# wei-zeng98/piano-a2s

Measured on AMD Instinct MI355X. Metric: training clips/sec (12 s, 5-bar), higher is better.
Workload: dtype f32

## Files before the change

### include/a2s.h

```cpp
#ifndef A2S_H
#define A2S_H
#include <stddef.h>
#include <stdint.h>
#ifdef __cplusplus
extern "C" {
#endif

#define A2S_OK 0
#define A2S_ERR_ARG (-1)
#define A2S_ERR_HIP (-2)
#define A2S_ERR_WORKSPACE (-3)

const char* a2s_last_error(void);
int a2s_version(void);
long long a2s_launch_count(void);

int a2s_gemm_f32(void* stream, int M, int N, int K, float alpha, const float* A, long sAm, long sAk,
                 const float* B, long sBk, long sBn, float beta, float* C, long ldc, const float* bias, int act,
                 int batch, long bsA, long bsB, long bsC, int splitk, float* workspace, size_t workspace_bytes);
int a2s_gemm_f32_affine(void* stream, int M, int N, int K, float alpha, const float* A, long sAm, long sAk, const float* B, long sBk,
                        long sBn, float beta, float* C, long ldc, const float* bias, int act, int batch, long bsA, long bsB, long bsC,
                        int splitk, float* workspace, size_t workspace_bytes, const float* a_scale, const float* a_shift, int a_period,
                        const float* b_scale, const float* b_shift, int b_period);
int a2s_gemm_f32_bnstats(void* stream, int M, int N, int K, const float* A, long sAm, long sAk, const float* B, long sBk, long sBn, float* C, long ldc,
// ... 14 lines not shown
int a2s_linear_wgrad(void* stream, int M, int N, int K, const float* dz, long ldz, const float* y, long lda, float* G, long ldg, const float* scale,
                     const float* shift, int period, const float* dz_absmax, const float* y_absmax, float* workspace, size_t workspace_bytes);
size_t a2s_linear_wgrad_ws_bytes(int M, int K);
int a2s_linear_wgrad_eligible(int M, int N, int K, int period);
size_t a2s_linear_dgrad_ws_bytes(int N, int K);
int a2s_linear_dgrad_blocks(int M);
int a2s_linear_dgrad_eligible(int M, int N, int K, int period);
int a2s_absmax(void* stream, const float* x, long n, float* out);
int a2s_gemm_bnstats_blocks(int M, int period);
size_t a2s_gemm_workspace_bytes(int M, int N, int batch, int splitk);
int a2s_gemm_pick_splitk(int M, int N, int K, int batch);
void a2s_gemm_debug_tile(int cfg);
int a2s_debug_set(const char* key, int value);
int a2s_debug_get(const char* key);
int a2s_env_check(void);
int a2s_persist_abort_latch(void* device_word);

int a2s_conv3x3(void* stream, const float* x, const float* w, float* y, const float* in_scale, const float* in_shift,
                float* stat_partial, int B, int T, int F, int Cin, int Cout, int flip, float* workspace);
int a2s_conv3x3_ranged(void* stream, const float* x, const float* w, float* y, const float* in_scale, const float* in_shift, const float* in_absmax,
                       float* stat_partial, float* out_absmax, int B, int T, int F, int Cin, int Cout, float* workspace);
int a2s_conv3x3_stat_blocks(int B, int T, int F, int Cin);
int a2s_conv3x3_dgrad_bnstats(void* stream, const float* dy, const float* w, float* g, const float* yl, const float* yl_mean, const float* yl_invstd,
                              const float* yl_scale, const float* yl_shift, float* stat_partial, int B, int T, int F, int Cin, int Cout,
                              float* workspace);
int a2s_bn_bwd_from_partial(void* stream, const float* g, const float* x, const float* mean, const float* invstd, const float* scale, const float* shift,
                            float* dgamma, float* dbeta, float* dx , const float* partial, int nblocks, float* c12, long rows, int C, int F);
int a2s_conv3x3_dgrad_bnstats_scaled(void* stream, const float* dy, const float* w, float* g, const float* yl, const float* yl_mean, const float* yl_invstd,
                                     const float* yl_scale, const float* yl_shift, float* stat_partial, int B, int T, int F, int Cin, int Cout,
                                     float* workspace, const float* dy_absmax);
// ... 182 lines not shown
```

### piano_a2s_amd/csrc/a2s_api.hip

```cpp
#define A2S_SWITCHES_IMPL
#include "a2s_internal.h"

thread_local char a2s_err_msg[512] = {0};
long long a2s_launch_counter = 0;

#define ST ((hipStream_t)stream)

extern "C" {

const char* a2s_last_error(void) { return a2s_err_msg; }
int a2s_version(void) { return 1; }
long long a2s_launch_count(void) { return __atomic_load_n(&a2s_launch_counter, __ATOMIC_RELAXED); }

int a2s_gemm_f32(void* stream, int M, int N, int K, float alpha, const float* A, long sAm, long sAk, const float* B, long sBk,
                 long sBn, float beta, float* C, long ldc, const float* bias, int act, int batch, long bsA, long bsB, long bsC,
                 int splitk, float* workspace, size_t workspace_bytes) {
    return a2s_gemm_impl(ST, M, N, K, alpha, A, sAm, sAk, B, sBk, sBn, beta, C, ldc, bias, act, batch, bsA, bsB, bsC, splitk,
                         workspace, workspace_bytes);
}
int a2s_gemm_f32_affine(void* stream, int M, int N, int K, float alpha, const float* A, long sAm, long sAk, const float* B, long sBk,
                        long sBn, float beta, float* C, long ldc, const float* bias, int act, int batch, long bsA, long bsB, long bsC,
                        int splitk, float* workspace, size_t workspace_bytes, const float* a_scale, const float* a_shift, int a_period,
                        const float* b_scale, const float* b_shift, int b_period) {
    return a2s_gemm_affine_impl(ST, M, N, K, alpha, A, sAm, sAk, B, sBk, sBn, beta, C, ldc, bias, act, batch, bsA, bsB, bsC, splitk,
// ... 40 lines not shown
int a2s_gemm_f32_bnstats(void* stream, int M, int N, int K, const float* A, long sAm, long sAk, const float* B, long sBk, long sBn, float* C, long ldc,
                         const float* y, const float* mean, const float* invstd, const float* scale, const float* shift, int period, float* partial) {
    return a2s_gemm_affine_impl(ST, M, N, K, 1.f, A, sAm, sAk, B, sBk, sBn, 0.f, C, ldc, nullptr, 0, 1, 0, 0, 0, 1, nullptr, 0,
                                nullptr, nullptr, 0, nullptr, nullptr, 0, y, mean, invstd, scale, shift, partial, period, 0, nullptr, nullptr);
}
int a2s_gemm_bnstats_blocks(int M, int period) { return a2s_cdiv(M, 128) * a2s_gemm_bnstats_slots(period); }
size_t a2s_gemm_workspace_bytes(int M, int N, int batch, int splitk) { return a2s_gemm_workspace_bytes_impl(M, N, batch, splitk); }
int a2s_gemm_pick_splitk(int M, int N, int K, int batch) { return a2s_gemm_pick_splitk_impl(M, N, K, batch); }
void a2s_gemm_debug_tile(int cfg) { a2s_gemm_debug_tile_impl(cfg); }
size_t a2s_note_step_workspace_floats(int H, int E) { return a2s_note_step_workspace_floats_impl(H, E); }
int a2s_debug_set(const char* key, int value) {
    if (!key) return A2S_ERR_ARG;
    const int id = a2s_switch_find(key);
    if (id >= 0) { a2s_switch_store(id, value); return A2S_OK; }
    if (!strcmp(key, "gemm_tile")) { a2s_gemm_debug_tile_impl(value); return A2S_OK; }
    snprintf(a2s_err_msg, sizeof(a2s_err_msg), "a2s_debug_set: unknown key %s", key);
    return A2S_ERR_ARG;
}
int a2s_env_check(void) {
    if (const char* e = a2s_switch_env_error()) A2S_FAIL(A2S_ERR_ARG, "%s: expected a decimal number >= 0", e);
    return A2S_OK;
}

int a2s_persist_abort_latch(void* device_word) { a2s_persist_latch_set(device_word); return A2S_OK; }

int a2s_debug_get(const char* key) {
    if (!key) return -1;
    const int id = a2s_switch_find(key);
    if (id == A2S_SW_attn_pair_fused_rows) return a2s_attn_pair_fused_rows();
    if (id >= 0) return a2s_sw((a2s_switch)id);
    if (!strcmp(key, "attn_pair_launches")) return (int)a2s_attn_pair_launches();
    if (!strcmp(key, "attn_pair_bwd_launches")) return (int)a2s_attn_pair_bwd_launches();
    if (!strcmp(key, "dec_mid_launches")) return a2s_dec_mid_launches();
    if (!strcmp(key, "dec_persist_launches")) return a2s_dec_persist_launches();
    if (!strcmp(key, "edit_distance_launches")) return (int)a2s_edit_distance_launches();
    if (!strcmp(key, "device_cus")) return a2s_device_geometry().cus;
    if (!strcmp(key, "device_xccs")) return a2s_device_geometry().xccs;
    return -1;
}

int a2s_conv3x3(void* stream, const float* x, const float* w, float* y, const float* in_scale, const float* in_shift,
                float* stat_partial, int B, int T, int F, int Cin, int Cout, int flip, float* workspace) {
    return a2s_conv3x3_impl(ST, x, w, y, in_scale, in_shift, stat_partial, B, T, F, Cin, Cout, flip, workspace, nullptr, nullptr, nullptr, nullptr, nullptr, nullptr,
                            nullptr, nullptr);
}
int a2s_conv3x3_ranged(void* stream, const float* x, const float* w, float* y, const float* in_scale, const float* in_shift, const float* in_absmax,
                       float* stat_partial, float* out_absmax, int B, int T, int F, int Cin, int Cout, float* workspace) {
    return a2s_conv3x3_impl(ST, x, w, y, in_scale, in_shift, stat_partial, B, T, F, Cin, Cout, 0, workspace, nullptr, nullptr, nullptr, nullptr, nullptr, nullptr,
// ... 243 lines not shown
```

### piano_a2s_amd/csrc/a2s_bwd.hip

```cpp
#include "a2s_internal.h"

__global__ __launch_bounds__(256) void log_softmax_bwd_rows(const float* __restrict__ g, const float* __restrict__ y,
                                                            long outer_stride, int inner, float* __restrict__ dx,
                                                            int R, int V, int n_outer, int time_major) {
    const int row = blockIdx.x * 4 + (threadIdx.x >> 6), lane = threadIdx.x & 63;
    if (row >= R) return;
    const int ob = row / inner, in = row % inner;
    const float* gr = g + (long)ob * outer_stride + (long)in * V;
    const float* yr = y + (long)ob * outer_stride + (long)in * V;
    float s = 0.f;
    for (int j = lane; j < V; j += 64) s += gr[j];
    s = wave_sum(s);
    const long orow = time_major ? ((long)in * n_outer + ob) : row;
    for (int j = lane; j < V; j += 64) dx[orow * V + j] = gr[j] - expf(yr[j]) * s;
}

int a2s_log_softmax_bwd_rows_impl(hipStream_t st, const float* g, const float* y, long outer_stride, int inner, float* dx,
                                  int R, int V, int n_outer, int time_major) {
    hipLaunchKernelGGL(log_softmax_bwd_rows, dim3(a2s_cdiv(R, 4)), dim3(256), 0, st, g, y, outer_stride, inner, dx, R, V, n_outer, time_major);
    A2S_CHECK_LAUNCH("log_softmax_bwd_rows");
    return A2S_OK;
}

__global__ void gru_gates_bwd(const float* __restrict__ dh_a, long lda, const float* __restrict__ dh_b, long ldb,
// ... 225 lines not shown

struct AttnPairBwdStep { const int* clip_order; const int* clip_rank; int n_clips; int n_active; int step; int G; int chunk; };
static int attn_pair_bwd_sweep(hipStream_t st, const a2s_note_dec_bwd_args& au, const a2s_note_dec_bwd_args& al, int s, AttnPairBwdStep& p);
static int attn_pair_bwd_combine(hipStream_t st, const a2s_note_dec_bwd_args& a, int s, const AttnPairBwdStep& p);

static int note_bwd_step_rows(const a2s_note_dec_bwd_args& a, int s) { return (a.row_list && a.n_rows_active) ? a.n_rows_active[s] : a.R; }
static thread_local int t_pair_rows_limit = -1;
struct PairRowsLimit { PairRowsLimit(int v) { t_pair_rows_limit = v; } ~PairRowsLimit() { t_pair_rows_limit = -1; } };
static bool note_bwd_step_fused(const a2s_note_dec_bwd_args& a, int s) {
    const void* ptrs[] = {a.dgi_all, a.dgh_all, a.dq_all, a.dx, a.dh, a.w_ih, a.w_hh, a.attn_w};
    const int n = note_bwd_step_rows(a, s);
    if (t_pair_rows_limit >= 0 && n > t_pair_rows_limit) return false;
    return n > 0 && a2s_dec_step_fusable(n, a.H, a.E, 173, ptrs, 8, a.step_ws, a.step_ws_floats);
}

static int note_bwd_step(hipStream_t st, const a2s_note_dec_bwd_args& a, int s, int& cur, bool mid, int part, const AttnPairBwdStep* pair) {
    const int H2 = 2 * a.H, ldx = a.E + H2, R = a.R;
    const bool fused = note_bwd_step_fused(a, s);
    a2s_attn_rows rows_v = {a.clip_order, a.clip_rank, a.row_until, a.n_clips > 0 ? a.n_clips : R, a.n_active ? a.n_active[s] : 0, s};
    const a2s_attn_rows* rows = a.n_active ? &rows_v : nullptr;
    float* dh_in = a.dh + (long)cur * R * H2;
    float* dh_out = a.dh + (long)(cur ^ 1) * R * H2;
    if (fused) {
        const int nrows = note_bwd_step_rows(a, s);
        int rc = a2s_note_step_fused_bwd(st, a, s, dh_in, dh_out, rows, nrows, nrows < R ? a.row_list : nullptr);
        if (rc) return rc;
        cur ^= 1;
        return A2S_OK;
    }
    int gM = R, gB = 1;
    long gS = 0;
    if (a.m_active && a.n_clips > 0 && a2s_prefix_rows_ok(a.m_active[s], a.n_clips)) { gM = a.m_active[s]; gB = R / a.n_clips; gS = a.n_clips; }
    const float* dos = a.do_all + (long)s * R * 2 * H2;
    float* dgi = a.dgi_all + (long)s * R * 3 * H2;
    float* dgh = a.dgh_all + (long)s * R * 3 * H2;
    float* dxs = a.dx + (long)s * R * ldx;
    int rc = A2S_OK;
    if (part != 2) {
        rc = a2s_gru_gates_bwd_impl(st, dh_in, H2, dos, 2 * H2, a.gates + (long)s * R * 4 * H2, a.h + (long)s * R * H2, H2,
                                    dgi, 3 * H2, dgh, 3 * H2, nullptr, 0, dh_out, H2, R, H2);
        if (rc) return rc;
        if (mid) {
            const int nrows = note_bwd_step_rows(a, s);
            rc = a2s_note_step_mid_bwd(st, a, s, dh_out, nrows, nrows < R ? a.row_list : nullptr);
        } else {
            rc = a2s_gemm_impl(st, gM, ldx, 3 * H2, 1.f, dgi, 3 * H2, 1, a.w_ih, ldx, 1, 0.f, dxs, ldx, nullptr, 0, gB, gS * 3 * H2, 0, gS * ldx, 0, a.gemm_ws, a.gemm_ws_bytes);
        }
        if (rc) return rc;
        if (part == 1) return A2S_OK;
    }
    rc = pair ? attn_pair_bwd_combine(st, a, s, *pair)
              : a2s_attn_step_bwd_impl(st, a.keys, a.enc, a.q + (long)s * R * a.H, a.H, a.attn_v, a.attw + (long)s * R * a.T,
                                       a.x + (long)s * R * ldx + a.E, ldx, dxs + a.E, ldx, dos + H2, 2 * H2,
                                       a.dctx_all + (long)s * R * H2, H2, a.dq_all + (long)s * R * a.H, a.H,
                                       a.ds_all + (long)s * R * a.T, R, a.T, a.H, a.attn_ws, rows);
    if (rc) return rc;
    if (!mid) {
        rc = a2s_gemm_impl(st, gM, H2, 3 * H2, 1.f, dgh, 3 * H2, 1, a.w_hh, H2, 1, 1.f, dh_out, H2, nullptr, 0, gB, gS * 3 * H2, 0, gS * H2, 0, a.gemm_ws, a.gemm_ws_bytes);
        if (rc) return rc;
    }
    if (mid) {
        const int nrows = note_bwd_step_rows(a, s);
        rc = a2s_note_step_mid_bwd_query(st, a, s, dh_out, nrows, nrows < R ? a.row_list : nullptr);
    } else
    rc = a2s_gemm_impl(st, gM, H2, a.H, 1.f, a.dq_all + (long)s * R * a.H, a.H, 1, a.attn_w, 2 * H2, 1, 1.f, dh_out, H2, nullptr, 0, gB, gS * a.H, 0, gS * H2, 0, a.gemm_ws, a.gemm_ws_bytes);
    if (rc) return rc;
    cur ^= 1;
    return A2S_OK;
}

static int note_bwd_prepare(hipStream_t st, const a2s_note_dec_bwd_args& a, bool* mid_out) {
    const int H2 = 2 * a.H, ldx = a.E + H2, R = a.R;
    hipError_t e = hipMemsetAsync(a.dh, 0, sizeof(float) * 2 * R * H2, st);
    if (e == hipSuccess && (a.m_active || a.row_list)) e = hipMemsetAsync(a.dx, 0, sizeof(float) * (size_t)a.steps * R * ldx, st);
    if (e != hipSuccess) A2S_FAIL(A2S_ERR_HIP, "note_decoder_bwd memset: %s", hipGetErrorString(e));
    bool any_fused = false;
    for (int s = a.steps - 1; s >= 0 && !any_fused; --s) any_fused = note_bwd_step_fused(a, s);
    const bool mid = a2s_note_step_mid_bwd_ok(a);
    bool any_mid = false;
    if (mid) for (int s = a.steps - 1; s >= 0 && !any_mid; --s) any_mid = !note_bwd_step_fused(a, s);
    if (any_fused || any_mid) { int rc = a2s_note_step_fused_bwd_prepare(st, a); if (rc) return rc; }
// ... 1 lines not shown
    return A2S_OK;
}
static int note_bwd_finish(hipStream_t st, const a2s_note_dec_bwd_args& a, int cur) {
    if (cur != 0) {
        const hipError_t e = hipMemcpyAsync(a.dh, a.dh + (long)a.R * 2 * a.H, sizeof(float) * a.R * 2 * a.H, hipMemcpyDeviceToDevice, st);
        if (e != hipSuccess) A2S_FAIL(A2S_ERR_HIP, "note_decoder_bwd copy: %s", hipGetErrorString(e));
    }
    return A2S_OK;
}

int a2s_note_decoder_bwd_impl(hipStream_t st, const a2s_note_dec_bwd_args& a) {
    if (a2s_note_decoder_bwd_persist_ok(a)) return a2s_note_decoder_bwd_persist(st, a);
    bool mid = false;
    int rc = note_bwd_prepare(st, a, &mid);
    if (rc) return rc;
    int cur = 0;
    for (int s = a.steps - 1; s >= 0; --s) {
        rc = note_bwd_step(st, a, s, cur, mid, 0, nullptr);
        if (rc) return rc;
    }
    return note_bwd_finish(st, a, cur);
}

int a2s_note_decoder_bwd_pair_impl(hipStream_t su, hipStream_t sl, const a2s_note_dec_bwd_args& au, const a2s_note_dec_bwd_args& al, const int* pair_order,
                                   const int* pair_rank, const int* pair_n_active) {
    const a2s_note_dec_bwd_args* as[2] = {&au, &al};
    hipStream_t sts[2] = {su, sl};
    const bool can_pair = a2s_sw(A2S_SW_attn_pair) && su != sl && pair_order && pair_rank && pair_n_active && au.n_active && al.n_active && au.n_clips > 0 &&
                          au.n_clips == al.n_clips && au.R == al.R && au.T == al.T && au.H == 256 && al.H == 256 && au.enc == al.enc && au.attn_ws && al.attn_ws &&
                          !a2s_note_decoder_bwd_persist_ok(au) && !a2s_note_decoder_bwd_persist_ok(al) && a2s_note_step_mid_bwd_ok(au) && a2s_note_step_mid_bwd_ok(al);
    if (!can_pair) {
        const int rc = a2s_note_decoder_bwd_impl(su, au);
        return rc ? rc : a2s_note_decoder_bwd_impl(sl, al);
    }
    static thread_local hipEvent_t ev[2] = {nullptr, nullptr};
    for (int k = 0; k < 2; ++k)
        if (!ev[k]) { const hipError_t e = hipEventCreateWithFlags(&ev[k], hipEventDisableTiming); if (e != hipSuccess) A2S_FAIL(A2S_ERR_HIP, "note_decoder_bwd_pair: hipEventCreate: %s", hipGetErrorString(e)); }
    bool mid[2] = {false, false};
    int cur[2] = {0, 0};
    const PairRowsLimit limit(a2s_attn_pair_fused_rows());
    for (int k = 0; k < 2; ++k) { const int rc = note_bwd_prepare(sts[k], *as[k], &mid[k]); if (rc) return rc; }
    const int nmax = au.steps > al.steps ? au.steps : al.steps;
    for (int s = nmax - 1; s >= 0; --s) {
        bool in[2], fused[2] = {false, false};
        for (int k = 0; k < 2; ++k) { in[k] = s < as[k]->steps; if (in[k]) fused[k] = note_bwd_step_fused(*as[k], s); }
        AttnPairBwdStep p = {pair_order, pair_rank, au.n_clips, pair_n_active[s], s, 1, au.T};
        const bool joint = in[0] && in[1] && mid[0] && mid[1] && !fused[0] && !fused[1] && p.n_active > 0 && au.n_active[s] > 0 && al.n_active[s] > 0;
        if (!joint) {
            for (int k = 0; k < 2; ++k)
                if (in[k]) { const int rc = note_bwd_step(sts[k], *as[k], s, cur[k], mid[k], 0, nullptr); if (rc) return rc; }
            continue;
        }
        for (int k = 0; k < 2; ++k) { const int rc = note_bwd_step(sts[k], *as[k], s, cur[k], mid[k], 1, nullptr); if (rc) return rc; }
        hipError_t e = hipEventRecord(ev[1], sl);
        if (e == hipSuccess) e = hipStreamWaitEvent(su, ev[1], 0);
        if (e != hipSuccess) A2S_FAIL(A2S_ERR_HIP, "note_decoder_bwd_pair: event: %s", hipGetErrorString(e));
        const int rc = attn_pair_bwd_sweep(su, au, al, s, p);
        if (rc) return rc;
        e = hipEventRecord(ev[0], su);
        if (e == hipSuccess) e = hipStreamWaitEvent(sl, ev[0], 0);
        if (e != hipSuccess) A2S_FAIL(A2S_ERR_HIP, "note_decoder_bwd_pair: event: %s", hipGetErrorString(e));
        for (int k = 0; k < 2; ++k) { const int rc2 = note_bwd_step(sts[k], *as[k], s, cur[k], mid[k], 2, &p); if (rc2) return rc2; }
    }
    for (int k = 0; k < 2; ++k) { const int rc = note_bwd_finish(sts[k], *as[k], cur[k]); if (rc) return rc; }
    return A2S_OK;
}


__global__ void transpose_f32(const float* __restrict__ in, float* __restrict__ out, int rows, int cols) {
    const int idx = blockIdx.x * blockDim.x + threadIdx.x;
    if (idx >= rows * cols) return;
    const int c = idx / rows, r = idx % rows;
    out[idx] = in[(long)r * cols + c];
}

int a2s_gru_seq_bwd_impl(hipStream_t st, const float* dout, long do_bstride, long do_tstride, const float* out, long out_bstride,
                         long out_tstride, const float* gates, const float* w_hh, const float* dhn, float* dgi_all, float* dgh_shift,
                         float* dgh_first, float* dhbuf, float* dgh_tmp, int B, int T, int H, int reverse, float* ws, size_t ws_bytes) {
    A2S_REQUIRE(dout && out && gates && w_hh && dgi_all && dgh_shift && dgh_first && dhbuf && dgh_tmp, "gru_seq_bwd: null tensor");
// ... 912 lines not shown
```

### piano_a2s_amd/csrc/a2s_internal.h

```cpp
#pragma once
#include "a2s_common.h"
#include "../../include/a2s.h"
#include "a2s_switches.h"

static inline int a2s_attn_pair_fused_rows(void) {
    const int cap = a2s_sw(A2S_SW_dec_fused_max_rows), v = a2s_sw(A2S_SW_attn_pair_fused_rows);
    return v < cap ? v : cap;
}
static inline unsigned a2s_persist_dbg(void) {
    return (a2s_sw(A2S_SW_persist_force_agent) ? PERSIST_DBG_FORCE_AGENT : 0u) | (a2s_sw(A2S_SW_persist_inject_abort) ? PERSIST_DBG_INJECT_ABORT : 0u);
}

int a2s_absmax_impl(hipStream_t st, const float* x, long n, float* out);
size_t a2s_gemm_workspace_bytes_impl(int M, int N, int batch, int splitk);
int a2s_gemm_pick_splitk_impl(int M, int N, int K, int batch);
int a2s_gemm_bnstats_slots(int period);
void a2s_gemm_debug_tile_impl(int cfg);
int a2s_gemm_affine_impl(hipStream_t st, int M, int N, int K, float alpha, const float* A, long sAm, long sAk,
    const float* B, long sBk, long sBn, float beta, float* C, long ldc, const float* bias, int act,
    int batch, long bsA, long bsB, long bsC, int splitk, float* ws, size_t ws_bytes,
    const float* a_scale, const float* a_shift, int a_period, const float* b_scale, const float* b_shift, int b_period,
    const float* ep_y, const float* ep_mean, const float* ep_invstd, const float* ep_scale, const float* ep_shift,
    float* ep_partial, int ep_period, int two_term, const float* a_absmax, const float* b_absmax);
int a2s_gemm_impl(hipStream_t st, int M, int N, int K, float alpha, const float* A, long sAm, long sAk,
// ... 108 lines not shown
int a2s_ew_act_bwd_impl(hipStream_t st, const float* g, const float* y, float* dx, long n, int act);
int a2s_note_decoder_bwd_impl(hipStream_t st, const a2s_note_dec_bwd_args& a);
int a2s_note_decoder_bwd_pair_impl(hipStream_t su, hipStream_t sl, const a2s_note_dec_bwd_args& au, const a2s_note_dec_bwd_args& al, const int* pair_order,
    const int* pair_rank, const int* pair_n_active);
int a2s_gru_seq_bwd_impl(hipStream_t st, const float* dout, long do_bstride, long do_tstride, const float* out, long out_bstride,
    long out_tstride, const float* gates, const float* w_hh, const float* dhn, float* dgi_all, float* dgh_shift,
    float* dgh_first, float* dhbuf, float* dgh_tmp, int B, int T, int H, int reverse, float* ws, size_t ws_bytes);
int a2s_staff_emb_bwd_impl(hipStream_t st, const float* note_emb, const float* const* w, float* const* grads_dev, float* note_emb_grad,
    const long long* ids64, const int* ids32, long id_bstride, const long long* lengths, long len_stride,
    const float* dout, long lddo, int col0, const float* hsave, int R, int maxlen, int E, int S);
long a2s_attn_pair_bwd_launches(void);

size_t a2s_note_step_fused_head_floats(void);
size_t a2s_note_step_workspace_floats_impl(int H, int E);
int a2s_dec_mid_launches(void);
bool a2s_dec_step_fusable(int R, int H, int E, int V, const void* const* ptrs, int nptrs, const float* ws, size_t ws_floats, bool greedy = false);
int a2s_note_step_fused_fwd(hipStream_t st, const a2s_note_dec_args& a, int si, int so, int sv, int sv_next, int t, const int* t_base, int tf, bool last,
    int nrows, const int* rowmap, const a2s_attn_deferred* defer = nullptr);
int a2s_note_step_fused_bwd_prepare(hipStream_t st, const a2s_note_dec_bwd_args& a);
int a2s_note_step_fused_bwd(hipStream_t st, const a2s_note_dec_bwd_args& a, int s, const float* dh_in, float* dh_out, const a2s_attn_rows* rows,
    int nrows, const int* rowmap);
bool a2s_note_step_mid_ok(int H, int E, const void* const* ptrs, int nptrs);
int a2s_note_step_mid_gru(hipStream_t st, const a2s_note_dec_args& a, int si, int so, int sv, int sv_next, int nrows, const int* rowmap);
bool a2s_note_step_mid_bwd_ok(const a2s_note_dec_bwd_args& a);
int a2s_note_step_mid_bwd(hipStream_t st, const a2s_note_dec_bwd_args& a, int s, float* dh_out, int nrows, const int* rowmap);
int a2s_note_step_mid_bwd_query(hipStream_t st, const a2s_note_dec_bwd_args& a, int s, float* dh_out, int nrows, const int* rowmap);

unsigned* a2s_persist_latch_ptr(void);
void a2s_persist_latch_set(void* p);
a2s_device_geom a2s_device_geometry(void);
bool a2s_gru_seq_fwd_persist_ok(const float* w_hh, const float* gi, int B, int T, int H, float* ws, size_t ws_bytes);
int a2s_gru_seq_fwd_persist_impl(hipStream_t st, const float* gi_all, long gi_bstride, long gi_tstride, const float* w_hh, const float* b_hh, float* out,
    long out_bstride, long out_tstride, float* save, float* hn, int B, int T, int H, int reverse, float* ws, size_t ws_bytes);
bool a2s_gru_seq_bwd_persist_ok(int B, int T, int H, float* ws, size_t ws_bytes, size_t ws_used);
int a2s_gru_seq_bwd_persist_impl(hipStream_t st, const float* dout, long do_bstride, long do_tstride, const float* out, long out_bstride, long out_tstride,
    const float* gates, const float* w_hh_t, const float* dhn, float* dgi_all, float* dgh_shift, float* dgh_first, int B, int T,
    int H, int reverse, float* ws, size_t ws_off, size_t ws_bytes);

int a2s_dec_persist_launches(void);
bool a2s_note_decoder_fwd_persist_ok(const a2s_note_dec_args& a);
int a2s_note_decoder_fwd_persist(hipStream_t st, const a2s_note_dec_args& a, int* steps_done);
// ... 18 lines not shown
```

### piano_a2s_amd/csrc/a2s_step.hip

```cpp
#include "a2s_internal.h"
#include <type_traits>

#define NW 8
#ifndef DEC_CH_GRU
#define DEC_CH_GRU 1
#define DEC_CH_OUT 1
#define DEC_CH_PROD 1
#define DEC_CH_QUERY 1
#endif
#ifndef DEC_NW_PROD
#define DEC_NW_PROD 8
#define DEC_NW_OUT 8
#endif

template <int NT, int CH, int NWV = NW>
__device__ __forceinline__ void mfma_rows8(const float* __restrict__ arow, const float* const (&brow)[NT], int ksteps, int wave, int lk,
                                           f32x4 (&acc)[NT]) {
    for (int u0 = wave; u0 < ksteps; u0 += NWV * CH) {
        f32x4 a[CH], b[NT][CH];
#pragma unroll
        for (int c = 0; c < CH; ++c) {
            const int u = u0 + NWV * c;
            const bool ok = u < ksteps;
            a[c] = ok ? *reinterpret_cast<const f32x4*>(arow + 16 * u + 4 * lk) : (f32x4){0.f, 0.f, 0.f, 0.f};
// ... 711 lines not shown
    f32x4 acc[2] = {(f32x4){0.f, 0.f, 0.f, 0.f}, (f32x4){0.f, 0.f, 0.f, 0.f}};
    mfma_rows8<2, DEC_CH_QUERY>(dq + (long)dec_row(rowmap, min(row0 + li, R - 1)) * H, brow, H / 16, wave, lk, acc);
    reduce_waves<2>(acc, part, wave, lane);
    if (wave > 0) return;
#pragma unroll
    for (int g = 0; g < 2; ++g) {
        const int col = n0 + g * 16 + li;
        if (col >= H2) continue;
#pragma unroll
        for (int r = 0; r < 4; ++r) {
            if (row0 + lk * 4 + r < R) dh[(long)dec_row(rowmap, row0 + lk * 4 + r) * H2 + col] = c0[g][r] + acc[g][r];
        }
    }
}

__global__ void transpose_ld(const float* __restrict__ in, long ld, float* __restrict__ out, int rows, int cols) {
    const long i = (long)blockIdx.x * blockDim.x + threadIdx.x;
    if (i >= (long)rows * cols) return;
    const int c = (int)(i / rows), r = (int)(i % rows);
    out[i] = in[(long)r * ld + c];
}

#define FUSED_MAX_ROWS_CAP 2048
#define FUSED_HEAD (16 + FUSED_MAX_ROWS_CAP / 16 + (long)FUSED_MAX_ROWS_CAP * 16 * NTV)
size_t a2s_note_step_fused_head_floats(void) { return (size_t)FUSED_HEAD; }
size_t a2s_note_step_workspace_floats_impl(int H, int E) {
    const long H2 = 2L * H, kx = E + H2;
    return (size_t)(FUSED_HEAD + kx * 3 * H2 + H2 * 3 * H2 + H2 * H);
}
static bool aligned16(const void* p) { return ((uintptr_t)p & 15) == 0; }
static int g_dec_mid_launches = 0;
int a2s_dec_mid_launches(void) { return g_dec_mid_launches; }
static bool dec_use_mid(int nrows, int H2) { return a2s_sw(A2S_SW_dec_mid) && nrows > 160 && H2 % MID_KC == 0; }
bool a2s_dec_step_fusable(int R, int H, int E, int V, const void* const* ptrs, int nptrs, const float* ws, size_t ws_floats, bool greedy) {
    const int max_rows = greedy ? FUSED_MAX_ROWS_CAP : a2s_sw(A2S_SW_dec_fused_max_rows);
    if (!a2s_sw(A2S_SW_dec_fused) || R > max_rows || R > FUSED_MAX_ROWS_CAP || !ws || ws_floats < a2s_note_step_workspace_floats_impl(H, E)) return false;
    if (H % 16 || E % 16 || (V + 15) / 16 != NTV || !aligned16(ws)) return false;
    for (int i = 0; i < nptrs; ++i) if (!aligned16(ptrs[i])) return false;
    return true;
}

int a2s_note_step_fused_fwd(hipStream_t st, const a2s_note_dec_args& a, int si, int so, int sv, int sv_next, int t, const int* t_base, int tf, bool last,
                            int nrows, const int* rowmap, const a2s_attn_deferred* defer) {
    const int H2 = 2 * a.H, ldx = a.E + H2, R = a.R;
    int* flags = reinterpret_cast<int*>(a.step_ws);
    const bool greedy = a.gt == nullptr;
    DecGruArgs g;
    g.x = a.x + (long)si * R * ldx; g.ldx = ldx; g.kx = ldx;
// ... 35 lines not shown
    return A2S_OK;
}

int a2s_note_step_fused_bwd_prepare(hipStream_t st, const a2s_note_dec_bwd_args& a) {
    const int H2 = 2 * a.H, kx = a.E + H2;
    float* wih_t = a.step_ws + FUSED_HEAD;
    float* whh_t = wih_t + (long)kx * 3 * H2;
    float* wh_t = whh_t + (long)H2 * 3 * H2;
    hipLaunchKernelGGL(transpose_ld, dim3(a2s_cdiv((long)3 * H2 * kx, 256)), dim3(256), 0, st, a.w_ih, (long)kx, wih_t, 3 * H2, kx);
    hipLaunchKernelGGL(transpose_ld, dim3(a2s_cdiv((long)3 * H2 * H2, 256)), dim3(256), 0, st, a.w_hh, (long)H2, whh_t, 3 * H2, H2);
    hipLaunchKernelGGL(transpose_ld, dim3(a2s_cdiv((long)a.H * H2, 256)), dim3(256), 0, st, a.attn_w, (long)2 * H2, wh_t, a.H, H2);
    A2S_CHECK_LAUNCH("transpose_ld");
    return A2S_OK;
}

int a2s_note_step_fused_bwd(hipStream_t st, const a2s_note_dec_bwd_args& a, int s, const float* dh_in, float* dh_out, const a2s_attn_rows* rows,
                            int nrows, const int* rowmap) {
    const int H2 = 2 * a.H, ldx = a.E + H2, R = a.R;
    const float* dos = a.do_all + (long)s * R * 2 * H2;
    float* dgi = a.dgi_all + (long)s * R * 3 * H2;
    float* dgh = a.dgh_all + (long)s * R * 3 * H2;
    float* dxs = a.dx + (long)s * R * ldx;
    float* wih_t = a.step_ws + FUSED_HEAD;
    float* whh_t = wih_t + (long)ldx * 3 * H2;
    float* wh_t = whh_t + (long)H2 * 3 * H2;
    DecBwdProdArgs p;
    p.dgi = dgi; p.dgh = dgh; p.wih_t = wih_t; p.whh_t = whh_t; p.dx = dxs; p.ldx = ldx; p.dh = dh_out;
    p.rowmap = rowmap;
    p.nxa = a2s_cdiv(ldx, 32); p.kx = ldx; p.R = nrows; p.H2 = H2;
    const bool mid = dec_use_mid(nrows, H2);
    int rc = a2s_gru_gates_bwd_impl(st, dh_in, H2, dos, 2 * H2, a.gates + (long)s * R * 4 * H2, a.h + (long)s * R * H2, H2,
                                    dgi, 3 * H2, dgh, 3 * H2, nullptr, 0, dh_out, H2, R, H2);
    if (rc) return rc;
    if (mid) { hipLaunchKernelGGL(dec_bwd_mid, dim3(p.nxa + a2s_cdiv(H2, 32), a2s_cdiv(nrows, 64)), dim3(256), 0, st, p); __atomic_fetch_add(&g_dec_mid_launches, 1, __ATOMIC_RELAXED); }
    else hipLaunchKernelGGL(dec_bwd_products, dim3(p.nxa + a2s_cdiv(H2, 32), a2s_cdiv(nrows, 16)), dim3(64 * DEC_NW_PROD), 0, st, p);
    A2S_CHECK_LAUNCH("dec_bwd_products");
    rc = a2s_attn_step_bwd_impl(st, a.keys, a.enc, a.q + (long)s * R * a.H, a.H, a.attn_v, a.attw + (long)s * R * a.T,
                                a.x + (long)s * R * ldx + a.E, ldx, dxs + a.E, ldx, dos + H2, 2 * H2,
                                a.dctx_all + (long)s * R * H2, H2, a.dq_all + (long)s * R * a.H, a.H,
                                a.ds_all + (long)s * R * a.T, R, a.T, a.H, a.attn_ws, rows);
    if (rc) return rc;
    if (mid) hipLaunchKernelGGL(dec_bwd_query_mid, dim3(a2s_cdiv(H2, 32), a2s_cdiv(nrows, 64)), dim3(256), 0, st, a.dq_all + (long)s * R * a.H, wh_t, dh_out, nrows, a.H, H2, rowmap);
    else hipLaunchKernelGGL(dec_bwd_query, dim3(a2s_cdiv(H2, 32), a2s_cdiv(nrows, 16)), dim3(64 * NW), 0, st, a.dq_all + (long)s * R * a.H, wh_t, dh_out, nrows, a.H, H2,
                            rowmap);
    A2S_CHECK_LAUNCH("dec_bwd_query");
    return A2S_OK;
}


bool a2s_note_step_mid_ok(int H, int E, const void* const* ptrs, int nptrs) {
    if (!a2s_sw(A2S_SW_dec_mid) || H % MID_KC || E % 16) return false;
    for (int i = 0; i < nptrs; ++i) if (!aligned16(ptrs[i])) return false;
    return true;
}
int a2s_note_step_mid_gru(hipStream_t st, const a2s_note_dec_args& a, int si, int so, int sv, int sv_next, int nrows, const int* rowmap) {
    const int H2 = 2 * a.H, ldx = a.E + H2, R = a.R;
// ... 25 lines not shown
}
int a2s_note_step_mid_bwd(hipStream_t st, const a2s_note_dec_bwd_args& a, int s, float* dh_out, int nrows, const int* rowmap) {
    const int H2 = 2 * a.H, ldx = a.E + H2, R = a.R;
    if (nrows <= 0) return A2S_OK;
    DecBwdProdArgs p;
    p.dgi = a.dgi_all + (long)s * R * 3 * H2; p.dgh = a.dgh_all + (long)s * R * 3 * H2;
    p.wih_t = a.step_ws + FUSED_HEAD; p.whh_t = p.wih_t + (long)ldx * 3 * H2;
    p.dx = a.dx + (long)s * R * ldx; p.ldx = ldx; p.dh = dh_out;
    p.rowmap = rowmap;
    p.nxa = a2s_cdiv(ldx, 32); p.kx = ldx; p.R = nrows; p.H2 = H2;
    hipLaunchKernelGGL(dec_bwd_mid, dim3(p.nxa + a2s_cdiv(H2, 32), a2s_cdiv(nrows, 64)), dim3(256), 0, st, p);
    __atomic_fetch_add(&g_dec_mid_launches, 1, __ATOMIC_RELAXED);
    A2S_CHECK_LAUNCH("dec_bwd_mid");
    return A2S_OK;
}
int a2s_note_step_mid_bwd_query(hipStream_t st, const a2s_note_dec_bwd_args& a, int s, float* dh_out, int nrows, const int* rowmap) {
    const int H2 = 2 * a.H, ldx = a.E + H2, R = a.R;
    if (nrows <= 0) return A2S_OK;
    const float* wh_t = a.step_ws + FUSED_HEAD + (long)ldx * 3 * H2 + (long)H2 * 3 * H2;
    hipLaunchKernelGGL(dec_bwd_query_mid, dim3(a2s_cdiv(H2, 32), a2s_cdiv(nrows, 64)), dim3(256), 0, st, a.dq_all + (long)s * R * a.H, wh_t, dh_out, nrows, a.H, H2, rowmap);
    A2S_CHECK_LAUNCH("dec_bwd_query_mid");
    return A2S_OK;
}
```

### piano_a2s_amd/hip.py

```python
import ctypes as C
import os

import torch

from .build import LIB

LIB = os.environ.get("A2S_LIB", LIB)

_lib = None


class A2SError(RuntimeError):
    pass


class NoteDecArgs(C.Structure):
    _fields_ = [(n, C.c_void_p) for n in (
        "attn_w", "attn_b", "attn_v", "w_ih", "w_hh", "b_ih", "b_hh", "out_w", "out_b", "emb", "keys", "enc",
        "h", "x", "q", "gates", "attw", "o", "gh", "gi", "logits")] + [
        ("probs", C.c_void_p), ("probs_bstride", C.c_long),
        ("gt", C.c_void_p), ("gt_bstride", C.c_long),
        ("tf_flags", C.c_void_p),
        ("drop", C.c_void_p), ("inv_keep", C.c_float),
        ("argmax_out", C.c_void_p), ("am_bstride", C.c_long),
# ... 24 lines not shown
            raise A2SError(f"HIP extension not built: {LIB} is missing (run `python __graft_entry__.py build`). "
                           "There is no CPU fallback for the transcription hot path.")
        arith = os.environ.get("A2S_ARITH", "f16x2")
        if arith not in ("f16x2", "bf16x3", "f32"):
            raise A2SError(f"A2S_ARITH={arith!r}: expected f16x2, bf16x3 or f32")
        L = C.CDLL(LIB)
        L.a2s_last_error.restype = C.c_char_p
        L.a2s_launch_count.restype = C.c_longlong
        for fn in ("a2s_note_step_workspace_floats", "a2s_note_decoder_persist_ws_bytes", "a2s_note_decoder_bwd_persist_ws_bytes", "a2s_linear_dgrad_ws_bytes", "a2s_linear_wgrad_ws_bytes", "a2s_gemm_workspace_bytes", "a2s_bn_bwd_partial_floats", "a2s_conv3x3_wgrad_workspace_bytes", "a2s_attn_workspace_floats", "a2s_attn_workspace_floats_fused",
                   "a2s_conv3x3_workspace_floats"):
            getattr(L, fn).restype = C.c_size_t
        if hasattr(L, "a2s_env_check") and L.a2s_env_check() != 0:
            raise A2SError(L.a2s_last_error().decode())
        if hasattr(L, "a2s_edit_distance"):
            L.a2s_edit_distance.argtypes = [C.c_void_p] * 6 + [C.c_int] * 3 + [C.c_void_p]
        if arith != "f16x2":
            for key in (b"conv_f16x2", b"wgrad_f16x2", b"gemm_f16x2"):
                L.a2s_debug_set(key, 0)
        if arith == "f32":
            for key in (b"conv_bf16x3", b"gemm_bf16x3", b"wgrad_bf16x3"):
                L.a2s_debug_set(key, 0)
        _lib = L
    return _lib


LINEAR_KERNELS = os.environ.get("A2S_LINEAR_KERNELS", "1") != "0"

_ABORT_LATCH = {}
PERSIST_ABORTS = 0

# ... 255 lines not shown
```

Measured before the change: 609.3.

## Fuse decoder backward query product with next step's GRU gate backward

Adds a tail kernel that runs the attention-query product into dh and then, in the same launch, computes the GRU cell backward for the previous step (s-1), writing dgi/dgh and the carried dh. The following step skips its separate gru_gates_bwd launch. This removes one kernel launch per decoder step and one round trip of dh through global memory in the sequential backward loop. In exchange it adds more complex kernels with a gate pass covering all R rows even when fewer rows are active, plus a new carry-buffer aliasing scheme. It is on by default behind a debug switch.

```diff
diff --git a/include/a2s.h b/include/a2s.h
--- a/include/a2s.h
+++ b/include/a2s.h
@@ -52,6 +52,7 @@
 int a2s_debug_set(const char* key, int value);
 int a2s_debug_get(const char* key);
 int a2s_env_check(void);
+int a2s_dec_bwd_tail_launches(void);
 int a2s_persist_abort_latch(void* device_word);
 
 int a2s_conv3x3(void* stream, const float* x, const float* w, float* y, const float* in_scale, const float* in_shift,
diff --git a/piano_a2s_amd/csrc/a2s_api.hip b/piano_a2s_amd/csrc/a2s_api.hip
--- a/piano_a2s_amd/csrc/a2s_api.hip
+++ b/piano_a2s_amd/csrc/a2s_api.hip
@@ -78,6 +78,7 @@
     const int id = a2s_switch_find(key);
     if (id >= 0) { a2s_switch_store(id, value); return A2S_OK; }
     if (!strcmp(key, "gemm_tile")) { a2s_gemm_debug_tile_impl(value); return A2S_OK; }
+    if (!strcmp(key, "dec_bwd_tail")) { a2s_dec_bwd_tail_set(value); return A2S_OK; }
     snprintf(a2s_err_msg, sizeof(a2s_err_msg), "a2s_debug_set: unknown key %s", key);
     return A2S_ERR_ARG;
 }
@@ -86,6 +87,7 @@
     return A2S_OK;
 }
 
+int a2s_dec_bwd_tail_launches(void) { return a2s_dec_bwd_tail_launches_impl(); }
 int a2s_persist_abort_latch(void* device_word) { a2s_persist_latch_set(device_word); return A2S_OK; }
 
 int a2s_debug_get(const char* key) {
@@ -96,6 +98,8 @@
     if (!strcmp(key, "attn_pair_launches")) return (int)a2s_attn_pair_launches();
     if (!strcmp(key, "attn_pair_bwd_launches")) return (int)a2s_attn_pair_bwd_launches();
     if (!strcmp(key, "dec_mid_launches")) return a2s_dec_mid_launches();
+    if (!strcmp(key, "dec_bwd_tail")) return a2s_dec_bwd_tail_on();
+    if (!strcmp(key, "dec_bwd_tail_launches")) return a2s_dec_bwd_tail_launches_impl();
     if (!strcmp(key, "dec_persist_launches")) return a2s_dec_persist_launches();
     if (!strcmp(key, "edit_distance_launches")) return (int)a2s_edit_distance_launches();
     if (!strcmp(key, "device_cus")) return a2s_device_geometry().cus;
diff --git a/piano_a2s_amd/csrc/a2s_bwd.hip b/piano_a2s_amd/csrc/a2s_bwd.hip
--- a/piano_a2s_amd/csrc/a2s_bwd.hip
+++ b/piano_a2s_amd/csrc/a2s_bwd.hip
@@ -263,8 +263,10 @@
     return n > 0 && a2s_dec_step_fusable(n, a.H, a.E, 173, ptrs, 8, a.step_ws, a.step_ws_floats);
 }
 
-static int note_bwd_step(hipStream_t st, const a2s_note_dec_bwd_args& a, int s, int& cur, bool mid, int part, const AttnPairBwdStep* pair) {
+struct NoteBwdLoop { int cur = 0; bool gated = false; bool tail = false; };
+static int note_bwd_step(hipStream_t st, const a2s_note_dec_bwd_args& a, int s, NoteBwdLoop& lp, bool mid, int part, const AttnPairBwdStep* pair) {
     const int H2 = 2 * a.H, ldx = a.E + H2, R = a.R;
+    int& cur = lp.cur;
     const bool fused = note_bwd_step_fused(a, s);
     a2s_attn_rows rows_v = {a.clip_order, a.clip_rank, a.row_until, a.n_clips > 0 ? a.n_clips : R, a.n_active ? a.n_active[s] : 0, s};
     const a2s_attn_rows* rows = a.n_active ? &rows_v : nullptr;
@@ -272,8 +274,9 @@
     float* dh_out = a.dh + (long)(cur ^ 1) * R * H2;
     if (fused) {
         const int nrows = note_bwd_step_rows(a, s);
-        int rc = a2s_note_step_fused_bwd(st, a, s, dh_in, dh_out, rows, nrows, nrows < R ? a.row_list : nullptr);
+        int rc = a2s_note_step_fused_bwd(st, a, s, dh_in, dh_out, rows, nrows, nrows < R ? a.row_list : nullptr, lp.gated, lp.tail);
         if (rc) return rc;
+        lp.gated = lp.tail && s > 0;
         cur ^= 1;
         return A2S_OK;
     }
@@ -286,8 +289,9 @@
     float* dxs = a.dx + (long)s * R * ldx;
     int rc = A2S_OK;
     if (part != 2) {
-        rc = a2s_gru_gates_bwd_impl(st, dh_in, H2, dos, 2 * H2, a.gates + (long)s * R * 4 * H2, a.h + (long)s * R * H2, H2,
-                                    dgi, 3 * H2, dgh, 3 * H2, nullptr, 0, dh_out, H2, R, H2);
+        if (!lp.gated)
+            rc = a2s_gru_gates_bwd_impl(st, dh_in, H2, dos, 2 * H2, a.gates + (long)s * R * 4 * H2, a.h + (long)s * R * H2, H2,
+                                        dgi, 3 * H2, dgh, 3 * H2, nullptr, 0, dh_out, H2, R, H2);
         if (rc) return rc;
         if (mid) {
             const int nrows = note_bwd_step_rows(a, s);
@@ -310,10 +314,11 @@
     }
     if (mid) {
         const int nrows = note_bwd_step_rows(a, s);
-        rc = a2s_note_step_mid_bwd_query(st, a, s, dh_out, nrows, nrows < R ? a.row_list : nullptr);
+        rc = a2s_note_step_mid_bwd_query(st, a, s, dh_out, dh_in, nrows, nrows < R ? a.row_list : nullptr, lp.tail);
     } else
     rc = a2s_gemm_impl(st, gM, H2, a.H, 1.f, a.dq_all + (long)s * R * a.H, a.H, 1, a.attn_w, 2 * H2, 1, 1.f, dh_out, H2, nullptr, 0, gB, gS * a.H, 0, gS * H2, 0, a.gemm_ws, a.gemm_ws_bytes);
     if (rc) return rc;
+    lp.gated = mid && lp.tail && s > 0;
     cur ^= 1;
     return A2S_OK;
 }
@@ -345,12 +350,13 @@
     bool mid = false;
     int rc = note_bwd_prepare(st, a, &mid);
     if (rc) return rc;
-    int cur = 0;
+    NoteBwdLoop lp;
+    lp.tail = a2s_dec_bwd_tail_on() != 0;
     for (int s = a.steps - 1; s >= 0; --s) {
-        rc = note_bwd_step(st, a, s, cur, mid, 0, nullptr);
+        rc = note_bwd_step(st, a, s, lp, mid, 0, nullptr);
         if (rc) return rc;
     }
-    return note_bwd_finish(st, a, cur);
+    return note_bwd_finish(st, a, lp.cur);
 }
 
 int a2s_note_decoder_bwd_pair_impl(hipStream_t su, hipStream_t sl, const a2s_note_dec_bwd_args& au, const a2s_note_dec_bwd_args& al, const int* pair_order,
@@ -368,7 +374,8 @@
     for (int k = 0; k < 2; ++k)
         if (!ev[k]) { const hipError_t e = hipEventCreateWithFlags(&ev[k], hipEventDisableTiming); if (e != hipSuccess) A2S_FAIL(A2S_ERR_HIP, "note_decoder_bwd_pair: hipEventCreate: %s", hipGetErrorString(e)); }
     bool mid[2] = {false, false};
-    int cur[2] = {0, 0};
+    NoteBwdLoop lp[2];
+    lp[0].tail = lp[1].tail = a2s_dec_bwd_tail_on() != 0;
     const PairRowsLimit limit(a2s_attn_pair_fused_rows());
     for (int k = 0; k < 2; ++k) { const int rc = note_bwd_prepare(sts[k], *as[k], &mid[k]); if (rc) return rc; }
     const int nmax = au.steps > al.steps ? au.steps : al.steps;
@@ -379,10 +386,10 @@
         const bool joint = in[0] && in[1] && mid[0] && mid[1] && !fused[0] && !fused[1] && p.n_active > 0 && au.n_active[s] > 0 && al.n_active[s] > 0;
         if (!joint) {
             for (int k = 0; k < 2; ++k)
-                if (in[k]) { const int rc = note_bwd_step(sts[k], *as[k], s, cur[k], mid[k], 0, nullptr); if (rc) return rc; }
+                if (in[k]) { const int rc = note_bwd_step(sts[k], *as[k], s, lp[k], mid[k], 0, nullptr); if (rc) return rc; }
             continue;
         }
-        for (int k = 0; k < 2; ++k) { const int rc = note_bwd_step(sts[k], *as[k], s, cur[k], mid[k], 1, nullptr); if (rc) return rc; }
+        for (int k = 0; k < 2; ++k) { const int rc = note_bwd_step(sts[k], *as[k], s, lp[k], mid[k], 1, nullptr); if (rc) return rc; }
         hipError_t e = hipEventRecord(ev[1], sl);
         if (e == hipSuccess) e = hipStreamWaitEvent(su, ev[1], 0);
         if (e != hipSuccess) A2S_FAIL(A2S_ERR_HIP, "note_decoder_bwd_pair: event: %s", hipGetErrorString(e));
@@ -391,9 +398,9 @@
         e = hipEventRecord(ev[0], su);
         if (e == hipSuccess) e = hipStreamWaitEvent(sl, ev[0], 0);
         if (e != hipSuccess) A2S_FAIL(A2S_ERR_HIP, "note_decoder_bwd_pair: event: %s", hipGetErrorString(e));
-        for (int k = 0; k < 2; ++k) { const int rc2 = note_bwd_step(sts[k], *as[k], s, cur[k], mid[k], 2, &p); if (rc2) return rc2; }
-    }
-    for (int k = 0; k < 2; ++k) { const int rc = note_bwd_finish(sts[k], *as[k], cur[k]); if (rc) return rc; }
+        for (int k = 0; k < 2; ++k) { const int rc2 = note_bwd_step(sts[k], *as[k], s, lp[k], mid[k], 2, &p); if (rc2) return rc2; }
+    }
+    for (int k = 0; k < 2; ++k) { const int rc = note_bwd_finish(sts[k], *as[k], lp[k].cur); if (rc) return rc; }
     return A2S_OK;
 }
 
diff --git a/piano_a2s_amd/csrc/a2s_internal.h b/piano_a2s_amd/csrc/a2s_internal.h
--- a/piano_a2s_amd/csrc/a2s_internal.h
+++ b/piano_a2s_amd/csrc/a2s_internal.h
@@ -146,17 +146,20 @@
 size_t a2s_note_step_fused_head_floats(void);
 size_t a2s_note_step_workspace_floats_impl(int H, int E);
 int a2s_dec_mid_launches(void);
+int a2s_dec_bwd_tail_on(void);
+void a2s_dec_bwd_tail_set(int on);
+int a2s_dec_bwd_tail_launches_impl(void);
 bool a2s_dec_step_fusable(int R, int H, int E, int V, const void* const* ptrs, int nptrs, const float* ws, size_t ws_floats, bool greedy = false);
 int a2s_note_step_fused_fwd(hipStream_t st, const a2s_note_dec_args& a, int si, int so, int sv, int sv_next, int t, const int* t_base, int tf, bool last,
     int nrows, const int* rowmap, const a2s_attn_deferred* defer = nullptr);
 int a2s_note_step_fused_bwd_prepare(hipStream_t st, const a2s_note_dec_bwd_args& a);
-int a2s_note_step_fused_bwd(hipStream_t st, const a2s_note_dec_bwd_args& a, int s, const float* dh_in, float* dh_out, const a2s_attn_rows* rows,
-    int nrows, const int* rowmap);
+int a2s_note_step_fused_bwd(hipStream_t st, const a2s_note_dec_bwd_args& a, int s, float* dh_in, float* dh_out, const a2s_attn_rows* rows,
+    int nrows, const int* rowmap, bool gated, bool tail);
 bool a2s_note_step_mid_ok(int H, int E, const void* const* ptrs, int nptrs);
 int a2s_note_step_mid_gru(hipStream_t st, const a2s_note_dec_args& a, int si, int so, int sv, int sv_next, int nrows, const int* rowmap);
 bool a2s_note_step_mid_bwd_ok(const a2s_note_dec_bwd_args& a);
 int a2s_note_step_mid_bwd(hipStream_t st, const a2s_note_dec_bwd_args& a, int s, float* dh_out, int nrows, const int* rowmap);
-int a2s_note_step_mid_bwd_query(hipStream_t st, const a2s_note_dec_bwd_args& a, int s, float* dh_out, int nrows, const int* rowmap);
+int a2s_note_step_mid_bwd_query(hipStream_t st, const a2s_note_dec_bwd_args& a, int s, float* dh_out, float* carry, int nrows, const int* rowmap, bool tail);
 
 unsigned* a2s_persist_latch_ptr(void);
 void a2s_persist_latch_set(void* p);
diff --git a/piano_a2s_amd/csrc/a2s_step.hip b/piano_a2s_amd/csrc/a2s_step.hip
--- a/piano_a2s_amd/csrc/a2s_step.hip
+++ b/piano_a2s_amd/csrc/a2s_step.hip
@@ -749,6 +749,112 @@
     }
 }
 
+struct DecBwdTailArgs {
+    const float* dq; const float* wh_t; float* dh;
+    const int* rowmap;
+    int nprod, R, H, H2;
+    int gate;
+    const float* dos; long lddo;
+    const float* save; const float* hprev;
+    float* dgi; float* dgh;
+    float* carry;
+};
+struct DecBwdTailCell { float rg, zg, ng, ghn, hp, dob; };
+__device__ __forceinline__ DecBwdTailCell dec_bwd_tail_load(const DecBwdTailArgs& a, long row, int col) {
+    const float* s = a.save + row * 4 * a.H2;
+    return DecBwdTailCell{s[col], s[a.H2 + col], s[2 * a.H2 + col], s[3 * a.H2 + col], a.hprev[row * a.H2 + col], a.dos[row * a.lddo + col]};
+}
+__device__ __forceinline__ void dec_bwd_tail_gate(const DecBwdTailArgs& a, long row, int col, float dh_out, const DecBwdTailCell& c) {
+    const int H2 = a.H2;
+    const float dh = dh_out + c.dob;
+    const GruCellGrad cg = gru_cell_bwd(dh, c.rg, c.zg, c.ng, c.ghn, c.hp);
+    float* gi = a.dgi + row * 3 * H2;
+    gi[col] = cg.dr; gi[H2 + col] = cg.dz; gi[2 * H2 + col] = cg.dn;
+    float* gh = a.dgh + row * 3 * H2;
+    gh[col] = cg.dr; gh[H2 + col] = cg.dz; gh[2 * H2 + col] = cg.dnr;
+    a.carry[row * H2 + col] = cg.dhz;
+}
+
+__global__ __launch_bounds__(256, MID_WAVES) void dec_bwd_tail_mid(DecBwdTailArgs a) {
+    __shared__ __attribute__((aligned(16))) float bs[2][32 * MID_LDB];
+    const int lane = threadIdx.x & 63, wave = threadIdx.x >> 6;
+    const int li = lane & 15, lk = lane >> 4;
+    const int H2 = a.H2, np = a.nprod;
+    const int row0 = blockIdx.y * 64 + wave * 16, n0 = blockIdx.x * 32;
+    const bool prod = (int)blockIdx.y * 64 < np;
+    f32x4 acc[2] = {(f32x4){0.f, 0.f, 0.f, 0.f}, (f32x4){0.f, 0.f, 0.f, 0.f}};
+    float c0[2][4];
+    if (prod) {
+#pragma unroll
+        for (int g = 0; g < 2; ++g)
+#pragma unroll
+            for (int r = 0; r < 4; ++r) c0[g][r] = a.dh[(long)dec_row(a.rowmap, min(row0 + lk * 4 + r, np - 1)) * H2 + min(n0 + g * 16 + li, H2 - 1)];
+        mid_product_64x32(a.dq + (long)dec_row(a.rowmap, min(row0 + li, np - 1)) * a.H + 4 * lk, a.wh_t, a.H, n0, H2, a.H, bs, acc);
+    }
+#pragma unroll
+    for (int g = 0; g < 2; ++g) {
+        const int col = n0 + g * 16 + li;
+        if (col >= H2) continue;
+#pragma unroll
+        for (int r = 0; r < 4; ++r) {
+            const int pos = row0 + lk * 4 + r;
+            if (pos >= (a.gate ? a.R : np)) continue;
+            const long row = dec_row(a.rowmap, pos);
+            float v;
+            if (pos < np) { v = c0[g][r] + acc[g][r]; a.dh[row * H2 + col] = v; }
+            else v = a.dh[row * H2 + col];
+            if (a.gate) dec_bwd_tail_gate(a, row, col, v, dec_bwd_tail_load(a, row, col));
+        }
+    }
+}
+
+__global__ __launch_bounds__(64 * NW) void dec_bwd_tail(DecBwdTailArgs a) {
+    __shared__ f32x4 part[4 * 2 * 64];
+    __shared__ float tile[16 * 32];
+    const int tid = threadIdx.x, lane = tid & 63, wave = tid >> 6;
+    const int li = lane & 15, lk = lane >> 4;
+    const int H = a.H, H2 = a.H2, np = a.nprod;
+    const int row0 = blockIdx.y * 16, n0 = blockIdx.x * 32;
+    const bool prod = row0 < np;
+    const int epos = row0 + (tid >> 5), ecol = n0 + (tid & 31);
+    const bool gate = a.gate && epos < a.R && ecol < H2;
+    const long erow = gate ? dec_row(a.rowmap, epos) : 0;
+    if (prod) {
+        const float* brow[2];
+#pragma unroll
+        for (int g = 0; g < 2; ++g) brow[g] = a.wh_t + (long)min(n0 + g * 16 + li, H2 - 1) * H;
+        float c0[2][4];
+        if (wave == 0) {
+#pragma unroll
+            for (int g = 0; g < 2; ++g)
+#pragma unroll
+                for (int r = 0; r < 4; ++r) c0[g][r] = a.dh[(long)dec_row(a.rowmap, min(row0 + lk * 4 + r, np - 1)) * H2 + min(n0 + g * 16 + li, H2 - 1)];
+        }
+        f32x4 acc[2] = {(f32x4){0.f, 0.f, 0.f, 0.f}, (f32x4){0.f, 0.f, 0.f, 0.f}};
+        mfma_rows8<2, DEC_CH_QUERY>(a.dq + (long)dec_row(a.rowmap, min(row0 + li, np - 1)) * H, brow, H / 16, wave, lk, acc);
+        reduce_waves<2>(acc, part, wave, lane);
+        if (wave == 0) {
+#pragma unroll
+            for (int g = 0; g < 2; ++g) {
+                const int col = n0 + g * 16 + li;
+#pragma unroll
+                for (int r = 0; r < 4; ++r) {
+                    const float v = c0[g][r] + acc[g][r];
+                    tile[(lk * 4 + r) * 32 + g * 16 + li] = v;
+                    if (col < H2 && row0 + lk * 4 + r < np) a.dh[(long)dec_row(a.rowmap, row0 + lk * 4 + r) * H2 + col] = v;
+                }
+            }
+        }
+    }
+    if (!a.gate) return;
+    DecBwdTailCell cell = {};
+    if (gate) cell = dec_bwd_tail_load(a, erow, ecol);
+    __syncthreads();
+    if (!gate) return;
+    const float v = epos < np ? tile[(tid >> 5) * 32 + (tid & 31)] : a.dh[erow * H2 + ecol];
+    dec_bwd_tail_gate(a, erow, ecol, v, cell);
+}
+
 __global__ void transpose_ld(const float* __restrict__ in, long ld, float* __restrict__ out, int rows, int cols) {
     const long i = (long)blockIdx.x * blockDim.x + threadIdx.x;
     if (i >= (long)rows * cols) return;
@@ -767,6 +873,11 @@
 static int g_dec_mid_launches = 0;
 int a2s_dec_mid_launches(void) { return g_dec_mid_launches; }
 static bool dec_use_mid(int nrows, int H2) { return a2s_sw(A2S_SW_dec_mid) && nrows > 160 && H2 % MID_KC == 0; }
+static int g_dec_bwd_tail = 1;
+static int g_dec_bwd_tail_launches = 0;
+int a2s_dec_bwd_tail_on(void) { return g_dec_bwd_tail; }
+void a2s_dec_bwd_tail_set(int on) { g_dec_bwd_tail = on ? 1 : 0; }
+int a2s_dec_bwd_tail_launches_impl(void) { return g_dec_bwd_tail_launches; }
 bool a2s_dec_step_fusable(int R, int H, int E, int V, const void* const* ptrs, int nptrs, const float* ws, size_t ws_floats, bool greedy) {
     const int max_rows = greedy ? FUSED_MAX_ROWS_CAP : a2s_sw(A2S_SW_dec_fused_max_rows);
     if (!a2s_sw(A2S_SW_dec_fused) || R > max_rows || R > FUSED_MAX_ROWS_CAP || !ws || ws_floats < a2s_note_step_workspace_floats_impl(H, E)) return false;
@@ -832,8 +943,29 @@
     return A2S_OK;
 }
 
-int a2s_note_step_fused_bwd(hipStream_t st, const a2s_note_dec_bwd_args& a, int s, const float* dh_in, float* dh_out, const a2s_attn_rows* rows,
-                            int nrows, const int* rowmap) {
+static int dec_bwd_tail_launch(hipStream_t st, const a2s_note_dec_bwd_args& a, int s, float* dh_out, float* carry, int nrows, const int* rowmap, bool gate, bool mid) {
+    const int H2 = 2 * a.H, R = a.R;
+    const int cover = gate ? R : nrows;
+    if (cover <= 0) return A2S_OK;
+    A2S_REQUIRE(!gate || (s > 0 && (rowmap || nrows == R)), "dec_bwd_tail: step %d of %d rows needs the call's row list for its gate part", s, nrows);
+    DecBwdTailArgs t = {};
+    t.dq = a.dq_all + (long)s * R * a.H; t.wh_t = a.step_ws + FUSED_HEAD + (long)(a.E + H2) * 3 * H2 + (long)H2 * 3 * H2; t.dh = dh_out;
+    t.rowmap = rowmap; t.nprod = nrows; t.R = R; t.H = a.H; t.H2 = H2; t.gate = gate ? 1 : 0;
+    if (gate) {
+        t.dos = a.do_all + (long)(s - 1) * R * 2 * H2; t.lddo = 2 * H2;
+        t.save = a.gates + (long)(s - 1) * R * 4 * H2; t.hprev = a.h + (long)(s - 1) * R * H2;
+        t.dgi = a.dgi_all + (long)(s - 1) * R * 3 * H2; t.dgh = a.dgh_all + (long)(s - 1) * R * 3 * H2;
+        t.carry = carry;
+        __atomic_fetch_add(&g_dec_bwd_tail_launches, 1, __ATOMIC_RELAXED);
+    }
+    if (mid) hipLaunchKernelGGL(dec_bwd_tail_mid, dim3(a2s_cdiv(H2, 32), a2s_cdiv(cover, 64)), dim3(256), 0, st, t);
+    else hipLaunchKernelGGL(dec_bwd_tail, dim3(a2s_cdiv(H2, 32), a2s_cdiv(cover, 16)), dim3(64 * NW), 0, st, t);
+    A2S_CHECK_LAUNCH("dec_bwd_tail");
+    return A2S_OK;
+}
+
+int a2s_note_step_fused_bwd(hipStream_t st, const a2s_note_dec_bwd_args& a, int s, float* dh_in, float* dh_out, const a2s_attn_rows* rows,
+                            int nrows, const int* rowmap, bool gated, bool tail) {
     const int H2 = 2 * a.H, ldx = a.E + H2, R = a.R;
     const float* dos = a.do_all + (long)s * R * 2 * H2;
     float* dgi = a.dgi_all + (long)s * R * 3 * H2;
@@ -847,8 +979,8 @@
     p.rowmap = rowmap;
     p.nxa = a2s_cdiv(ldx, 32); p.kx = ldx; p.R = nrows; p.H2 = H2;
     const bool mid = dec_use_mid(nrows, H2);
-    int rc = a2s_gru_gates_bwd_impl(st, dh_in, H2, dos, 2 * H2, a.gates + (long)s * R * 4 * H2, a.h + (long)s * R * H2, H2,
-                                    dgi, 3 * H2, dgh, 3 * H2, nullptr, 0, dh_out, H2, R, H2);
+    int rc = gated ? A2S_OK : a2s_gru_gates_bwd_impl(st, dh_in, H2, dos, 2 * H2, a.gates + (long)s * R * 4 * H2, a.h + (long)s * R * H2, H2,
+                                                     dgi, 3 * H2, dgh, 3 * H2, nullptr, 0, dh_out, H2, R, H2);
     if (rc) return rc;
     if (mid) { hipLaunchKernelGGL(dec_bwd_mid, dim3(p.nxa + a2s_cdiv(H2, 32), a2s_cdiv(nrows, 64)), dim3(256), 0, st, p); __atomic_fetch_add(&g_dec_mid_launches, 1, __ATOMIC_RELAXED); }
     else hipLaunchKernelGGL(dec_bwd_products, dim3(p.nxa + a2s_cdiv(H2, 32), a2s_cdiv(nrows, 16)), dim3(64 * DEC_NW_PROD), 0, st, p);
@@ -858,6 +990,7 @@
                                 a.dctx_all + (long)s * R * H2, H2, a.dq_all + (long)s * R * a.H, a.H,
                                 a.ds_all + (long)s * R * a.T, R, a.T, a.H, a.attn_ws, rows);
     if (rc) return rc;
+    if (tail) return dec_bwd_tail_launch(st, a, s, dh_out, dh_in, nrows, rowmap, s > 0, mid);
     if (mid) hipLaunchKernelGGL(dec_bwd_query_mid, dim3(a2s_cdiv(H2, 32), a2s_cdiv(nrows, 64)), dim3(256), 0, st, a.dq_all + (long)s * R * a.H, wh_t, dh_out, nrows, a.H, H2, rowmap);
     else hipLaunchKernelGGL(dec_bwd_query, dim3(a2s_cdiv(H2, 32), a2s_cdiv(nrows, 16)), dim3(64 * NW), 0, st, a.dq_all + (long)s * R * a.H, wh_t, dh_out, nrows, a.H, H2,
                             rowmap);
@@ -913,8 +1046,9 @@
     A2S_CHECK_LAUNCH("dec_bwd_mid");
     return A2S_OK;
 }
-int a2s_note_step_mid_bwd_query(hipStream_t st, const a2s_note_dec_bwd_args& a, int s, float* dh_out, int nrows, const int* rowmap) {
+int a2s_note_step_mid_bwd_query(hipStream_t st, const a2s_note_dec_bwd_args& a, int s, float* dh_out, float* carry, int nrows, const int* rowmap, bool tail) {
     const int H2 = 2 * a.H, ldx = a.E + H2, R = a.R;
+    if (tail) return dec_bwd_tail_launch(st, a, s, dh_out, carry, nrows, rowmap, s > 0, true);
     if (nrows <= 0) return A2S_OK;
     const float* wh_t = a.step_ws + FUSED_HEAD + (long)ldx * 3 * H2 + (long)H2 * 3 * H2;
     hipLaunchKernelGGL(dec_bwd_query_mid, dim3(a2s_cdiv(H2, 32), a2s_cdiv(nrows, 64)), dim3(256), 0, st, a.dq_all + (long)s * R * a.H, wh_t, dh_out, nrows, a.H, H2, rowmap);
diff --git a/piano_a2s_amd/hip.py b/piano_a2s_amd/hip.py
--- a/piano_a2s_amd/hip.py
+++ b/piano_a2s_amd/hip.py
@@ -62,6 +62,9 @@
             raise A2SError(L.a2s_last_error().decode())
         if hasattr(L, "a2s_edit_distance"):
             L.a2s_edit_distance.argtypes = [C.c_void_p] * 6 + [C.c_int] * 3 + [C.c_void_p]
+        if hasattr(L, "a2s_dec_bwd_tail_launches"):
+            L.a2s_dec_bwd_tail_launches.restype = C.c_int
+            L.a2s_dec_bwd_tail_launches.argtypes = []
         if arith != "f16x2":
             for key in (b"conv_f16x2", b"wgrad_f16x2", b"gemm_f16x2"):
                 L.a2s_debug_set(key, 0)
```

Result: no change. 611.4 (median of 6 runs) (+0.3%).
